# chenxuhao/GraphMiner

Measured on AMD Instinct MI355X. Metric: million edges processed/sec + total match count, higher is better.
Workload: dtype int32 (vertex ids, offsets; uint64 counts); 1 GPU; tc: triangle counting, LiveJournal stand-in; graph=rmat_s22_ef10_seed42, nv=4194304, ne_sym=81171116, tasks=40585558, max_degree=777, parallelism=task-chunk round-robin x1, replicated CSR

## Files before the change

graphminer_amd/csrc/gm_tch.hip:

```cpp
#include <type_traits>
#include "gm_flat.h"

namespace gm {

#ifndef GM_TCH_TILES
#define GM_TCH_TILES 4
#endif
constexpr int kTchTiles = GM_TCH_TILES;
#ifndef GM_TCH_TILES_SMALL
#define GM_TCH_TILES_SMALL 2
#endif
constexpr int kTchTilesSmall = GM_TCH_TILES_SMALL;
constexpr int kTchFlatTilesSmall = 4, kTchFlatTilesBig = 8;

#ifndef GM_TCH_LONG_LIST
#define GM_TCH_LONG_LIST 384
#endif
constexpr int kTchLongList = GM_TCH_LONG_LIST;

constexpr int kTchOvfCap = 128;
constexpr unsigned kTchEmpty = 0xffffffffu, kTchMarker = 0xfffffffeu;
constexpr unsigned kTchMul = 0x9E3779B1u;

template <int BITWIN>
struct alignas(16) TchWave {
  int2 desc[GM_WAVE];
  unsigned bits[BITWIN / 32 + 8];
};

#ifndef GM_TCH_WAVES_BIG
#define GM_TCH_WAVES_BIG 4
#endif
#ifndef GM_TCH_MIN_WG_BIG
#define GM_TCH_MIN_WG_BIG 4
#endif
template <int STAGE>
constexpr int tch_waves() { return STAGE <= 1024 ? kWavesPerBlock : GM_TCH_WAVES_BIG; }
template <int STAGE>
struct alignas(16) TchLds {
  uint4 table[STAGE];
  int rpl[kMaxChunkVerts + 1];
  int trpl[kMaxChunkVerts + 1];
  static constexpr int kBitWindow = STAGE <= 1024 ? 8192 : 4096;
  TchWave<kBitWindow> w[tch_waves<STAGE>()];
  int ovf_key[kTchOvfCap];
  int ovf_salt[kTchOvfCap];
  int n_ovf;
  int next_batch;
  unsigned queue_pos;
  int next_group;
};
static_assert(kTchOvfCap == 2 * GM_WAVE, "the surplus list is scanned two entries per lane");

template <int STAGE>
struct TchHash {
  static constexpr int LB = STAGE == 1024 ? 10 : 11;
  static_assert((1 << LB) == STAGE, "one bucket per stage entry");
  static constexpr unsigned kMask = (unsigned)(STAGE - 1) << 4;
  static __device__ __forceinline__ unsigned bucket(int x, unsigned s) { return ((((unsigned)x * kTchMul) >> (28 - LB)) & kMask) ^ s; }
  static __device__ __forceinline__ unsigned salt(int local_row) { return (((unsigned)local_row * 37u) & (unsigned)(STAGE - 1)) << 4; }
  static __device__ __forceinline__ int row_of(unsigned s) { return (int)(((s >> 4) * 941u) & (unsigned)(STAGE - 1)); }
};

__device__ __forceinline__ int tch_local_row(const int *rpl, const int nvl, const int e) {
  int lo = 0, hi = nvl - 1;
  while (lo < hi) {
    const int mid = (lo + hi + 1) >> 1;
    if (rpl[mid] <= e) lo = mid; else hi = mid - 1;
  }
  return lo;
}

template <int STAGE, int T>
__device__ __forceinline__ void tch_probe(const TchLds<STAGE> &B, const int *__restrict__ col, const bool fallback, const int (&key)[T],
                                          const unsigned (&salt)[T], const unsigned long long (&inm)[T], unsigned long long (&hm)[T],
                                          unsigned long long (&nm)[T]) {
  if (fallback) {
#pragma unroll
    for (int q = 0; q < T; ++q) {
      bool f = false;
      if (__builtin_amdgcn_inverse_ballot_w64(inm[q])) {
        const int lo = TchHash<STAGE>::row_of(salt[q]);
        const int rs = B.rpl[lo], rn = B.rpl[lo + 1] - rs;
        const int pos = lower_bound(col + rs, rn, key[q]);
        f = pos < rn && col[rs + pos] == key[q];
      }
      hm[q] = __ballot(f);
      nm[q] = 0ull;
    }
    return;
  }
  uint4 w[T];
#pragma unroll
  for (int q = 0; q < T; ++q)
    w[q] = *reinterpret_cast<const uint4 *>(reinterpret_cast<const char *>(B.table) + TchHash<STAGE>::bucket(key[q], salt[q]));
#pragma unroll
  for (int q = 0; q < T; ++q) {
    const unsigned k = (unsigned)key[q];
    const unsigned long long m = __ballot(w[q].x == k) | __ballot(w[q].y == k) | __ballot(w[q].z == k) | __ballot(w[q].w == k);
    hm[q] = m & inm[q];
    nm[q] = __ballot(w[q].w == kTchMarker) & ~m & inm[q];
  }
}

template <int STAGE, int T>
__device__ __forceinline__ unsigned tch_surplus(const TchLds<STAGE> &B, const int lane, const int (&key)[T], const unsigned (&salt)[T],
                                                const unsigned long long (&nm)[T]) {
  const int k0 = B.ovf_key[lane], k1 = B.ovf_key[lane + GM_WAVE];
  const int s0 = B.ovf_salt[lane], s1 = B.ovf_salt[lane + GM_WAVE];
  unsigned c = 0;
#pragma unroll
  for (int q = 0; q < T; ++q) {
    unsigned long long rest = nm[q];
    while (rest) {
      const int src = __ffsll((long long)rest) - 1;
      rest &= rest - 1;
      const int k = readlane(key[q], src), s = readlane((int)salt[q], src);
      if (__ballot(((k0 == k) & (s0 == s)) | ((k1 == k) & (s1 == s))) != 0ull) ++c;
    }
  }
  return c;
}

template <int STAGE>
__device__ __forceinline__ unsigned tch_pass(TchLds<STAGE> &B, TchWave<TchLds<STAGE>::kBitWindow> &L, const int *__restrict__ col, const bool fallback, const int lane,
                                             const int llen_all, const int key_base, const unsigned salt_l) {
  constexpr int T = STAGE <= 1024 ? kTchTilesSmall : kTchTiles;
  constexpr int TF = STAGE <= 1024 ? kTchFlatTilesSmall : kTchFlatTilesBig;
  unsigned cnt = 0;
  if (wave_max_nonneg(llen_all) == 0) return 0u;
  const bool is_long = llen_all >= kTchLongList;
  const int llen = is_long ? 0 : llen_all;

  unsigned long long lm = __ballot(is_long);
  while (lm) {
    const int src = __ffsll((long long)lm) - 1;
    lm &= lm - 1;
    const int base = readlane(key_base, src);
    const int n = readlane(llen_all, src);
    const unsigned s_u = (unsigned)readlane((int)salt_l, src);
    const int *__restrict__ kp = col + base;
    auto process = [&](auto kc, const int (&key)[T], const unsigned long long (&inm)[T]) {
      constexpr int K = decltype(kc)::value;
      int k2[K];
      unsigned salt[K];
      unsigned long long i2[K], hm[K], nm[K];
#pragma unroll
      for (int q = 0; q < K; ++q) {
        k2[q] = key[q];
        salt[q] = s_u;
        i2[q] = inm[q];
      }
      tch_probe<STAGE, K>(B, col, fallback, k2, salt, i2, hm, nm);
      unsigned long long any_need = 0ull;
#pragma unroll
      for (int q = 0; q < K; ++q) {
        cnt += (unsigned)__popcll(hm[q]);
        any_need |= nm[q];
      }
      if (any_need != 0ull) cnt += tch_surplus<STAGE, K>(B, lane, k2, salt, nm);
    };
    constexpr int G = GM_WAVE * T;
    int nxt[T];
#pragma unroll
    for (int q = 0; q < T; ++q) nxt[q] = kp[min(q * GM_WAVE + lane, n - 1)];
    int t = 0;
    for (; t + 2 * G <= n; t += G) {
      int key[T];
      unsigned long long inm[T];
#pragma unroll
      for (int q = 0; q < T; ++q) {
        key[q] = nxt[q];
        inm[q] = ~0ull;
      }
      const int *__restrict__ kn = kp + (t + G);
#pragma unroll
      for (int q = 0; q < T; ++q) nxt[q] = kn[(unsigned)(q * GM_WAVE + lane)];
      process(std::integral_constant<int, T>{}, key, inm);
    }
    for (; t < n; t += G) {
      int key[T];
      unsigned long long inm[T];
#pragma unroll
      for (int q = 0; q < T; ++q) {
        key[q] = nxt[q];
        inm[q] = __ballot((t + q * GM_WAVE + lane) < n);
      }
#pragma unroll
      for (int q = 0; q < T; ++q) nxt[q] = kp[min(t + G + q * GM_WAVE + lane, n - 1)];
      const int tiles = min(T, (n - t + GM_WAVE - 1) >> 6);
      if (tiles >= T) process(std::integral_constant<int, T>{}, key, inm);
      else if (tiles == 1) process(std::integral_constant<int, 1>{}, key, inm);
      else if constexpr (T > 2) {
        if (tiles == 2) process(std::integral_constant<int, 2>{}, key, inm);
        else process(std::integral_constant<int, (T > 2 ? 3 : 1)>{}, key, inm);
      }
    }
  }

  const int incl = wave_incl_scan_add(llen);
  const int total = readlane(incl, GM_WAVE - 1);
  if (total == 0) return cnt;
  const int off = incl - llen;
  const unsigned long long nzm = __ballot(llen > 0);
  if (llen > 0) L.desc[rank_below(nzm)] = make_int2(key_base - off, (int)salt_l);
  constexpr int G = GM_WAVE * TF, kBitWin = TchLds<STAGE>::kBitWindow;
  constexpr int TH = 4, NH = TF / TH;
  static_assert(TF % TH == 0, "tile groups are made of half-groups of four");
  struct Grp {
    int key[NH][TH];
    unsigned salt[NH][TH];
    unsigned long long inm[NH][TH];
  };
  for (int wb = 0; wb < total; wb += kBitWin) {
    const int wn = min(kBitWin, total - wb);
    const int nw = ((wn + G - 1) / G) * (G / 32) + 2;
    for (int i = lane; i < nw; i += GM_WAVE) L.bits[i] = 0u;
    wave_sync();
    if (llen > 0 && off > wb && off < wb + kBitWin) atomicOr(&L.bits[(off - 1 - wb) >> 5], 1u << ((off - 1 - wb) & 31));
    int carry = __popcll(__ballot(llen > 0 && off <= wb)) - 1;
    wave_sync();
    auto stage_a = [&](const int g, Grp &r) {
      int2 d[TF];
      bool in[TF];
      const int mw = (int)L.bits[((g * G) >> 5) + (lane & (2 * TF - 1))];
#pragma unroll
      for (int q = 0; q < TF; ++q) {
        const unsigned long long m = ((unsigned long long)(unsigned)readlane(mw, 2 * q + 1) << 32) | (unsigned)readlane(mw, 2 * q);
        const int own = carry + rank_below(m);
        carry += __popcll(m);
        in[q] = (wb + g * G + q * GM_WAVE + lane) < total;
        r.inm[q / TH][q % TH] = __ballot(in[q]);
        d[q] = L.desc[in[q] ? own : 0];
      }
#pragma unroll
      for (int q = 0; q < TF; ++q) {
        r.key[q / TH][q % TH] = col[in[q] ? d[q].x + (wb + g * G + q * GM_WAVE + lane) : 0];
        r.salt[q / TH][q % TH] = (unsigned)d[q].y;
      }
    };
    auto stage_b = [&](const Grp &r) {
#pragma unroll
      for (int h = 0; h < NH; ++h) {
        unsigned long long hm[TH], nm[TH];
        tch_probe<STAGE, TH>(B, col, fallback, r.key[h], r.salt[h], r.inm[h], hm, nm);
        unsigned long long any_need = 0ull;
#pragma unroll
        for (int q = 0; q < TH; ++q) {
          cnt += (unsigned)__popcll(hm[q]);
          any_need |= nm[q];
        }
        if (any_need != 0ull) cnt += tch_surplus<STAGE, TH>(B, lane, r.key[h], r.salt[h], nm);
      }
    };
    const int ng = (wn + G - 1) / G;
    Grp cur;
    stage_a(0, cur);
    for (int g = 0; g + 1 < ng; ++g) {
      Grp nxt;
      stage_a(g + 1, nxt);
      stage_b(cur);
      cur = nxt;
    }
    stage_b(cur);
    wave_sync();
  }
  return cnt;
}

#ifndef GM_TCH_MIN_WG
#define GM_TCH_MIN_WG 6
#endif
template <int STAGE>
__global__ __launch_bounds__((tch_waves<STAGE>() * GM_WAVE), (STAGE <= 1024 ? GM_TCH_MIN_WG : GM_TCH_MIN_WG_BIG))
void tch_kernel(const MineParams p) {
  __shared__ TchLds<STAGE> B;
  using H = TchHash<STAGE>;
  const int lane = threadIdx.x & (GM_WAVE - 1);
  const int wave = threadIdx.x >> 6;
  constexpr int nthreads = tch_waves<STAGE>() * GM_WAVE;
  const int tid = threadIdx.x;
  const int *__restrict__ rp = p.g.rp;
  const int *__restrict__ col = p.g.col;
  const int *__restrict__ trp = p.g.trp;
  const int2 *__restrict__ tdesc = p.g.tdesc;
  auto &L = B.w[wave];
  unsigned long long c0 = 0;
  for (;;) {
    if (tid == 0) B.queue_pos = atomicAdd(p.queue, (unsigned)p.grab);
    __syncthreads();
    const unsigned q = B.queue_pos;
    if (q >= (unsigned)p.count) break;
    const unsigned qe = min(q + (unsigned)p.grab, (unsigned)p.count);
    constexpr int kU = 4;
    auto chunk_at = [&](const unsigned ci) {
      const size_t pos = (size_t)p.first + (size_t)ci * (size_t)p.step;
      return p.chunks[p.order ? (size_t)p.order[pos] : pos];
    };
    ChunkRec rn = chunk_at(q);
    bool have_pre = false;
    int xn[kU], rpn = 0, trpn = 0;
    for (unsigned ci = q; ci < qe; ++ci) {
      const ChunkRec r = rn;
      const int ub = r.u_begin, nvl = r.u_end - r.u_begin;
      const int eb = r.e_begin, nel = r.e_end - r.e_begin;
      unsigned *fill32 = reinterpret_cast<unsigned *>(&B.w[0]);
      if (have_pre) {
        if (tid <= nvl) {
          B.rpl[tid] = rpn;
          B.trpl[tid] = trpn;
        }
        for (int i = tid + nthreads; i <= nvl; i += nthreads) {
          B.rpl[i] = rp[ub + i];
          B.trpl[i] = trp[ub + i];
        }
      } else {
        for (int i = tid; i <= nvl; i += nthreads) {
          B.rpl[i] = rp[ub + i];
          B.trpl[i] = trp[ub + i];
        }
      }
      {
        const uint4 empty = make_uint4(kTchEmpty, kTchEmpty, kTchEmpty, kTchEmpty);
        for (int i = tid; i < STAGE; i += nthreads) B.table[i] = empty;
        for (int i = tid; i < STAGE / 2; i += nthreads) fill32[i] = 0u;
        if (tid < kTchOvfCap) {
          B.ovf_key[tid] = -1;
          B.ovf_salt[tid] = -1;
        }
        if (tid == 0) {
          B.n_ovf = 0;
          B.next_batch = 0;
          B.next_group = 0;
        }
      }
      __syncthreads();
      unsigned *slots = reinterpret_cast<unsigned *>(B.table);
      for (int i0 = tid; i0 < nel; i0 += kU * nthreads) {
        int x[kU];
        if (have_pre && i0 == tid) {
#pragma unroll
          for (int j = 0; j < kU; ++j) x[j] = xn[j];
        } else {
#pragma unroll
          for (int j = 0; j < kU; ++j) x[j] = col[eb + min(i0 + j * nthreads, nel - 1)];
        }
#pragma unroll
        for (int j = 0; j < kU; ++j) {
          const int i = i0 + j * nthreads;
          if (i < nel) {
            const unsigned s = H::salt(tch_local_row(B.rpl, nvl, eb + i));
            const unsigned b = H::bucket(x[j], s) >> 4;
            const unsigned shift = (b & 1u) * 16u;
            const unsigned slot = (atomicAdd(&fill32[b >> 1], 1u << shift) >> shift) & 0xffffu;
            if (slot < 4u) {
              slots[(b << 2) + slot] = (unsigned)x[j];
            } else {
              const int jo = atomicAdd(&B.n_ovf, 1);
              if (jo < kTchOvfCap) {
                B.ovf_key[jo] = x[j];
                B.ovf_salt[jo] = (int)s;
              }
            }
          }
        }
      }
      __syncthreads();
      for (int b = tid; b < STAGE; b += nthreads) {
        const unsigned c = (fill32[b >> 1] >> ((b & 1) * 16)) & 0xffffu;
        if (c > 4u) {
          const unsigned x3 = slots[(b << 2) + 3];
          const int jo = atomicAdd(&B.n_ovf, 1);
          if (jo < kTchOvfCap) {
            B.ovf_key[jo] = (int)x3;
            B.ovf_salt[jo] = (int)(H::bucket((int)x3, 0u) ^ ((unsigned)b << 4));
          }
          slots[(b << 2) + 3] = kTchMarker;
        }
      }
      __syncthreads();
      const bool fallback = B.n_ovf > kTchOvfCap || (p.flags & (1 << 22)) != 0;
      have_pre = ci + 1 < qe;
      if (have_pre) {
        rn = chunk_at(ci + 1);
        const int nel_n = rn.e_end - rn.e_begin, nvl_n = rn.u_end - rn.u_begin;
#pragma unroll
        for (int j = 0; j < kU; ++j) xn[j] = col[rn.e_begin + min(tid + j * nthreads, max(nel_n - 1, 0))];
        rpn = rp[rn.u_begin + min(tid, nvl_n)];
        trpn = trp[rn.u_begin + min(tid, nvl_n)];
      }
      if (p.g.kst != nullptr) {
        constexpr int TS = 4, GS = TS * GM_WAVE;
        const int kb = p.g.kst_rp[ub], kn = p.g.kst_rp[ub + nvl] - kb;
        const unsigned *__restrict__ kp = p.g.kst + kb;
        auto grab = [&]() {
          int gi = 0;
          if (lane == 0) gi = atomicAdd(&B.next_group, 1);
          return (readfirst(gi) * r.nparts + r.part) * GS;
        };
        unsigned nxt[TS];
        int g0 = kn > 0 ? grab() : 0;
        if (g0 < kn) {
#pragma unroll
          for (int q = 0; q < TS; ++q) nxt[q] = kp[min(g0 + q * GM_WAVE + lane, kn - 1)];
        }
        while (g0 < kn) {
          const int gc = g0;
          int key[TS];
          unsigned salt[TS];
          unsigned long long inm[TS], hm[TS], nm[TS];
#pragma unroll
          for (int q = 0; q < TS; ++q) {
            key[q] = (int)(nxt[q] & 0xffffffu);
            salt[q] = H::salt((int)(((nxt[q] >> 24) - (unsigned)ub) & 255u));
            inm[q] = __ballot(gc + q * GM_WAVE + lane < kn);
          }
          g0 = grab();
          if (g0 < kn) {
#pragma unroll
            for (int q = 0; q < TS; ++q) nxt[q] = kp[min(g0 + q * GM_WAVE + lane, kn - 1)];
          }
          tch_probe<STAGE, TS>(B, col, fallback, key, salt, inm, hm, nm);
          unsigned long long any_need = 0ull;
          unsigned cnt = 0;
#pragma unroll
          for (int q = 0; q < TS; ++q) {
            cnt += (unsigned)__popcll(hm[q]);
            any_need |= nm[q];
          }
          if (any_need != 0ull) cnt += tch_surplus<STAGE, TS>(B, lane, key, salt, nm);
          c0 += (unsigned long long)cnt;
        }
      }
      const int tb = B.trpl[0], ntask = B.trpl[nvl] - tb;
      for (;;) {
        int bi = 0;
        if (lane == 0) bi = atomicAdd(&B.next_batch, 1);
        bi = readfirst(bi) * r.nparts + r.part;
        const int t0 = bi * GM_WAVE;
        if (t0 >= ntask) break;
        const bool valid = t0 + lane < ntask;
        const int te = tb + min(t0 + lane, ntask - 1);
        const int2 d = tdesc[te];
        const int lo = tch_local_row(B.trpl, nvl, te);
        const int ru = B.rpl[lo], a = B.rpl[lo + 1] - ru;
        const bool act = valid && d.y > 0 && a > 0;
        c0 += (unsigned long long)tch_pass<STAGE>(B, L, col, fallback, lane, act ? d.y : 0, d.x, H::salt(lo));
      }
      __syncthreads();
    }
  }
  if (lane == 0 && c0) atomicAdd(&p.counters[0], c0);
}

int tch_per_cu(int stage) {
  if (stage <= 1024) return 6;
  return (int)std::max<size_t>(1, std::min<size_t>(163840 / sizeof(TchLds<kTctStageMax>), 2048 / (tch_waves<kTctStageMax>() * GM_WAVE)));
}
hipError_t launch_tch(const MineParams &p, int stage, int grid_blocks, hipStream_t stream) {
  static_assert(sizeof(TchLds<1024>) * 6 <= 163840, "six workgroups per CU");
  static_assert(sizeof(TchLds<kTctStageMax>) <= 163840, "one workgroup per CU at least");
  static_assert(sizeof(TchWave<4096>) * tch_waves<kTctStageMax>() >= (size_t)kTctStageMax * 2, "fill counters alias the wave scratch");
  if (p.g.trp == nullptr || p.g.tdesc == nullptr) return hipErrorInvalidValue;
  const dim3 grid((unsigned)grid_blocks);
  if (stage <= 1024) hipLaunchKernelGGL((tch_kernel<1024>), grid, dim3(kWavesPerBlock * GM_WAVE), 0, stream, p);
  else hipLaunchKernelGGL((tch_kernel<kTctStageMax>), grid, dim3(tch_waves<kTctStageMax>() * GM_WAVE), 0, stream, p);
  return hipGetLastError();
}

}

__global__ void gm_touch_tch_kernel() {}
void gm_touch_tch() { hipLaunchKernelGGL(gm_touch_tch_kernel, dim3(1), dim3(1), 0, 0); }
```

Before: 23930 Medges/s.

## Precompute hash buckets, narrow 32-bit col offsets, and drop per-lane bounds checks in TC probes

Callers now pass precomputed LDS bucket offsets to the probe, and the salt is redefined as the global host id, so tagged keys map straight to a bucket without per-key salt arithmetic. A NARROW template variant, used when the edge count fits in 29 bits, keeps column offsets as biased 32-bit byte offsets instead of 64-bit addresses. Descriptor lookup uses mbcnt directly, and only the final partial tile group is guarded. The flat loop is unrolled into two ping-pong buffers, and the key-group prefetch skips clamping for full groups. This lowers VALU and address work per probe, at the cost of more kernel instantiations and trickier offset and bias arithmetic.

Result: slower. 20080 Medges/s (-16.1%).

```diff
diff --git a/graphminer_amd/csrc/gm_tch.hip b/graphminer_amd/csrc/gm_tch.hip
--- a/graphminer_amd/csrc/gm_tch.hip
+++ b/graphminer_amd/csrc/gm_tch.hip
@@ -58,8 +58,12 @@
   static_assert((1 << LB) == STAGE, "one bucket per stage entry");
   static constexpr unsigned kMask = (unsigned)(STAGE - 1) << 4;
   static __device__ __forceinline__ unsigned bucket(int x, unsigned s) { return ((((unsigned)x * kTchMul) >> (28 - LB)) & kMask) ^ s; }
-  static __device__ __forceinline__ unsigned salt(int local_row) { return (((unsigned)local_row * 37u) & (unsigned)(STAGE - 1)) << 4; }
-  static __device__ __forceinline__ int row_of(unsigned s) { return (int)(((s >> 4) * 941u) & (unsigned)(STAGE - 1)); }
+  static constexpr int kSaltShift = LB - 4;
+  static __device__ __forceinline__ unsigned salt(int host) { return ((unsigned)host & 255u) << kSaltShift; }
+  static __device__ __forceinline__ int row_of(unsigned s, int ub) { return (int)(((s >> kSaltShift) - (unsigned)ub) & 255u); }
+  static __device__ __forceinline__ unsigned bucket_tagged(unsigned w) {
+    return ((((w & 0xffffffu) * kTchMul) ^ (w & 0xff000000u)) >> (28 - LB)) & kMask;
+  }
 };
 
 __device__ __forceinline__ int tch_local_row(const int *rpl, const int nvl, const int e) {
@@ -72,15 +76,15 @@
 }
 
 template <int STAGE, int T>
-__device__ __forceinline__ void tch_probe(const TchLds<STAGE> &B, const int *__restrict__ col, const bool fallback, const int (&key)[T],
-                                          const unsigned (&salt)[T], const unsigned long long (&inm)[T], unsigned long long (&hm)[T],
+__device__ __forceinline__ void tch_probe(const TchLds<STAGE> &B, const int *__restrict__ col, const bool fallback, const int ub, const int (&key)[T],
+                                          const unsigned (&bkt)[T], const unsigned long long (&inm)[T], unsigned long long (&hm)[T],
                                           unsigned long long (&nm)[T]) {
   if (fallback) {
 #pragma unroll
     for (int q = 0; q < T; ++q) {
       bool f = false;
       if (__builtin_amdgcn_inverse_ballot_w64(inm[q])) {
-        const int lo = TchHash<STAGE>::row_of(salt[q]);
+        const int lo = TchHash<STAGE>::row_of(bkt[q] ^ TchHash<STAGE>::bucket(key[q], 0u), ub);
         const int rs = B.rpl[lo], rn = B.rpl[lo + 1] - rs;
         const int pos = lower_bound(col + rs, rn, key[q]);
         f = pos < rn && col[rs + pos] == key[q];
@@ -92,8 +96,7 @@
   }
   uint4 w[T];
 #pragma unroll
-  for (int q = 0; q < T; ++q)
-    w[q] = *reinterpret_cast<const uint4 *>(reinterpret_cast<const char *>(B.table) + TchHash<STAGE>::bucket(key[q], salt[q]));
+  for (int q = 0; q < T; ++q) w[q] = *reinterpret_cast<const uint4 *>(reinterpret_cast<const char *>(B.table) + bkt[q]);
 #pragma unroll
   for (int q = 0; q < T; ++q) {
     const unsigned k = (unsigned)key[q];
@@ -104,7 +107,7 @@
 }
 
 template <int STAGE, int T>
-__device__ __forceinline__ unsigned tch_surplus(const TchLds<STAGE> &B, const int lane, const int (&key)[T], const unsigned (&salt)[T],
+__device__ __forceinline__ unsigned tch_surplus(const TchLds<STAGE> &B, const int lane, const int (&key)[T], const unsigned (&bkt)[T],
                                                 const unsigned long long (&nm)[T]) {
   const int k0 = B.ovf_key[lane], k1 = B.ovf_key[lane + GM_WAVE];
   const int s0 = B.ovf_salt[lane], s1 = B.ovf_salt[lane + GM_WAVE];
@@ -115,16 +118,17 @@
     while (rest) {
       const int src = __ffsll((long long)rest) - 1;
       rest &= rest - 1;
-      const int k = readlane(key[q], src), s = readlane((int)salt[q], src);
+      const int k = readlane(key[q], src);
+      const int s = (int)((unsigned)readlane((int)bkt[q], src) ^ TchHash<STAGE>::bucket(k, 0u));
       if (__ballot(((k0 == k) & (s0 == s)) | ((k1 == k) & (s1 == s))) != 0ull) ++c;
     }
   }
   return c;
 }
 
-template <int STAGE>
-__device__ __forceinline__ unsigned tch_pass(TchLds<STAGE> &B, TchWave<TchLds<STAGE>::kBitWindow> &L, const int *__restrict__ col, const bool fallback, const int lane,
-                                             const int llen_all, const int key_base, const unsigned salt_l) {
+template <int STAGE, bool NARROW>
+__device__ __forceinline__ unsigned tch_pass(TchLds<STAGE> &B, TchWave<TchLds<STAGE>::kBitWindow> &L, const int *__restrict__ col, const bool fallback, const int ub,
+                                             const int lane, const int llen_all, const int key_base, const unsigned salt_l) {
   constexpr int T = STAGE <= 1024 ? kTchTilesSmall : kTchTiles;
   constexpr int TF = STAGE <= 1024 ? kTchFlatTilesSmall : kTchFlatTilesBig;
   unsigned cnt = 0;
@@ -143,22 +147,22 @@
     auto process = [&](auto kc, const int (&key)[T], const unsigned long long (&inm)[T]) {
       constexpr int K = decltype(kc)::value;
       int k2[K];
-      unsigned salt[K];
+      unsigned bk[K];
       unsigned long long i2[K], hm[K], nm[K];
 #pragma unroll
       for (int q = 0; q < K; ++q) {
         k2[q] = key[q];
-        salt[q] = s_u;
+        bk[q] = TchHash<STAGE>::bucket(key[q], s_u);
         i2[q] = inm[q];
       }
-      tch_probe<STAGE, K>(B, col, fallback, k2, salt, i2, hm, nm);
+      tch_probe<STAGE, K>(B, col, fallback, ub, k2, bk, i2, hm, nm);
       unsigned long long any_need = 0ull;
 #pragma unroll
       for (int q = 0; q < K; ++q) {
         cnt += (unsigned)__popcll(hm[q]);
         any_need |= nm[q];
       }
-      if (any_need != 0ull) cnt += tch_surplus<STAGE, K>(B, lane, k2, salt, nm);
+      if (any_need != 0ull) cnt += tch_surplus<STAGE, K>(B, lane, k2, bk, nm);
     };
     constexpr int G = GM_WAVE * T;
     int nxt[T];
@@ -203,8 +207,10 @@
   if (total == 0) return cnt;
   const int off = incl - llen;
   const unsigned long long nzm = __ballot(llen > 0);
-  if (llen > 0) L.desc[rank_below(nzm)] = make_int2(key_base - off, (int)salt_l);
   constexpr int G = GM_WAVE * TF, kBitWin = TchLds<STAGE>::kBitWindow;
+  constexpr unsigned kBias = (unsigned)(GM_WAVE * (TF - 1)) << 2;
+  if (llen > 0) L.desc[rank_below(nzm)] = make_int2(NARROW ? (int)(((unsigned)(key_base - off) << 2) + kBias) : key_base - off, (int)salt_l);
+  const char *__restrict__ cbase = reinterpret_cast<const char *>(col) - kBias;
   constexpr int TH = 4, NH = TF / TH;
   static_assert(TF % TH == 0, "tile groups are made of half-groups of four");
   struct Grp {
@@ -212,6 +218,7 @@
     unsigned salt[NH][TH];
     unsigned long long inm[NH][TH];
   };
+  const unsigned lane4 = (unsigned)lane << 2;
   for (int wb = 0; wb < total; wb += kBitWin) {
     const int wn = min(kBitWin, total - wb);
     const int nw = ((wn + G - 1) / G) * (G / 32) + 2;
@@ -222,47 +229,74 @@
     wave_sync();
     auto stage_a = [&](const int g, Grp &r) {
       int2 d[TF];
-      bool in[TF];
+      const int p0 = wb + g * G;
       const int mw = (int)L.bits[((g * G) >> 5) + (lane & (2 * TF - 1))];
 #pragma unroll
       for (int q = 0; q < TF; ++q) {
-        const unsigned long long m = ((unsigned long long)(unsigned)readlane(mw, 2 * q + 1) << 32) | (unsigned)readlane(mw, 2 * q);
-        const int own = carry + rank_below(m);
-        carry += __popcll(m);
-        in[q] = (wb + g * G + q * GM_WAVE + lane) < total;
-        r.inm[q / TH][q % TH] = __ballot(in[q]);
-        d[q] = L.desc[in[q] ? own : 0];
-      }
+        const unsigned mlo = (unsigned)readlane(mw, 2 * q), mhi = (unsigned)readlane(mw, 2 * q + 1);
+        const int2 *dp = L.desc + carry;
+        d[q] = dp[__builtin_amdgcn_mbcnt_hi(mhi, __builtin_amdgcn_mbcnt_lo(mlo, 0u))];
+        carry += __popc(mlo) + __popc(mhi);
+        r.salt[q / TH][q % TH] = (unsigned)d[q].y;
+        r.inm[q / TH][q % TH] = ~0ull;
+      }
+      using Off = std::conditional_t<NARROW, unsigned, long long>;
+      Off o[TF];
 #pragma unroll
       for (int q = 0; q < TF; ++q) {
-        r.key[q / TH][q % TH] = col[in[q] ? d[q].x + (wb + g * G + q * GM_WAVE + lane) : 0];
-        r.salt[q / TH][q % TH] = (unsigned)d[q].y;
+        if constexpr (NARROW) o[q] = (unsigned)d[q].x + (lane4 + (unsigned)(p0 << 2));
+        else o[q] = (long long)d[q].x + (long long)(p0 + q * GM_WAVE + lane);
+      }
+      if (p0 + G > total) {
+        asm volatile("; guarded tile group");
+#pragma unroll
+        for (int q = 0; q < TF; ++q) {
+          const int n = max(min(total - (p0 + q * GM_WAVE), GM_WAVE), 0);
+          const unsigned long long m = n >= GM_WAVE ? ~0ull : ((1ull << n) - 1ull);
+          r.inm[q / TH][q % TH] = m;
+          o[q] = __builtin_amdgcn_inverse_ballot_w64(m) ? o[q] : (Off)(NARROW ? kBias - (unsigned)(q * GM_WAVE * 4) : 0u);
+        }
+      }
+#pragma unroll
+      for (int q = 0; q < TF; ++q) {
+        if constexpr (NARROW) r.key[q / TH][q % TH] = *reinterpret_cast<const int *>(cbase + (size_t)o[q] + (size_t)(q * GM_WAVE * 4));
+        else r.key[q / TH][q % TH] = col[o[q]];
       }
     };
     auto stage_b = [&](const Grp &r) {
 #pragma unroll
       for (int h = 0; h < NH; ++h) {
+        unsigned bk[TH];
         unsigned long long hm[TH], nm[TH];
-        tch_probe<STAGE, TH>(B, col, fallback, r.key[h], r.salt[h], r.inm[h], hm, nm);
+#pragma unroll
+        for (int q = 0; q < TH; ++q) bk[q] = TchHash<STAGE>::bucket(r.key[h][q], r.salt[h][q]);
+        tch_probe<STAGE, TH>(B, col, fallback, ub, r.key[h], bk, r.inm[h], hm, nm);
         unsigned long long any_need = 0ull;
 #pragma unroll
         for (int q = 0; q < TH; ++q) {
           cnt += (unsigned)__popcll(hm[q]);
           any_need |= nm[q];
         }
-        if (any_need != 0ull) cnt += tch_surplus<STAGE, TH>(B, lane, r.key[h], r.salt[h], nm);
+        if (any_need != 0ull) cnt += tch_surplus<STAGE, TH>(B, lane, r.key[h], bk, nm);
       }
     };
     const int ng = (wn + G - 1) / G;
-    Grp cur;
-    stage_a(0, cur);
-    for (int g = 0; g + 1 < ng; ++g) {
-      Grp nxt;
-      stage_a(g + 1, nxt);
-      stage_b(cur);
-      cur = nxt;
+    Grp ga, gb;
+    stage_a(0, ga);
+    for (int g = 0;; g += 2) {
+      if (g + 1 >= ng) {
+        stage_b(ga);
+        break;
+      }
+      stage_a(g + 1, gb);
+      stage_b(ga);
+      if (g + 2 >= ng) {
+        stage_b(gb);
+        break;
+      }
+      stage_a(g + 2, ga);
+      stage_b(gb);
     }
-    stage_b(cur);
     wave_sync();
   }
   return cnt;
@@ -271,13 +305,13 @@
 #ifndef GM_TCH_MIN_WG
 #define GM_TCH_MIN_WG 6
 #endif
-template <int STAGE>
+template <int STAGE, bool NARROW>
 __global__ __launch_bounds__((tch_waves<STAGE>() * GM_WAVE), (STAGE <= 1024 ? GM_TCH_MIN_WG : GM_TCH_MIN_WG_BIG))
 void tch_kernel(const MineParams p) {
   __shared__ TchLds<STAGE> B;
   using H = TchHash<STAGE>;
   const int lane = threadIdx.x & (GM_WAVE - 1);
-  const int wave = threadIdx.x >> 6;
+  const int wave = readfirst((int)(threadIdx.x >> 6));
   constexpr int nthreads = tch_waves<STAGE>() * GM_WAVE;
   const int tid = threadIdx.x;
   const int *__restrict__ rp = p.g.rp;
@@ -349,7 +383,7 @@
         for (int j = 0; j < kU; ++j) {
           const int i = i0 + j * nthreads;
           if (i < nel) {
-            const unsigned s = H::salt(tch_local_row(B.rpl, nvl, eb + i));
+            const unsigned s = H::salt(ub + tch_local_row(B.rpl, nvl, eb + i));
             const unsigned b = H::bucket(x[j], s) >> 4;
             const unsigned shift = (b & 1u) * 16u;
             const unsigned slot = (atomicAdd(&fill32[b >> 1], 1u << shift) >> shift) & 0xffffu;
@@ -399,28 +433,44 @@
           return (readfirst(gi) * r.nparts + r.part) * GS;
         };
         unsigned nxt[TS];
-        int g0 = kn > 0 ? grab() : 0;
-        if (g0 < kn) {
-#pragma unroll
-          for (int q = 0; q < TS; ++q) nxt[q] = kp[min(g0 + q * GM_WAVE + lane, kn - 1)];
+        auto request = [&](const int g) {
+          if (g + GS <= kn) {
+            const unsigned *__restrict__ kg = kp + g;
+#pragma unroll
+            for (int q = 0; q < TS; ++q) nxt[q] = kg[(unsigned)(q * GM_WAVE + lane)];
+          } else {
+#pragma unroll
+            for (int q = 0; q < TS; ++q) nxt[q] = kp[min(g + q * GM_WAVE + lane, kn - 1)];
+            asm volatile("; guarded tile group");
+          }
+        };
+        int g0 = kn;
+        if (kn > 0) {
+          g0 = grab();
+          request(g0);
         }
         while (g0 < kn) {
           const int gc = g0;
           int key[TS];
-          unsigned salt[TS];
+          unsigned bk[TS];
           unsigned long long inm[TS], hm[TS], nm[TS];
 #pragma unroll
           for (int q = 0; q < TS; ++q) {
             key[q] = (int)(nxt[q] & 0xffffffu);
-            salt[q] = H::salt((int)(((nxt[q] >> 24) - (unsigned)ub) & 255u));
-            inm[q] = __ballot(gc + q * GM_WAVE + lane < kn);
+            bk[q] = H::bucket_tagged(nxt[q]);
+            inm[q] = ~0ull;
+          }
+          if (gc + GS > kn) {
+            asm volatile("; guarded tile group");
+#pragma unroll
+            for (int q = 0; q < TS; ++q) {
+              const int n = max(min(kn - (gc + q * GM_WAVE), GM_WAVE), 0);
+              inm[q] = n >= GM_WAVE ? ~0ull : ((1ull << n) - 1ull);
+            }
           }
           g0 = grab();
-          if (g0 < kn) {
-#pragma unroll
-            for (int q = 0; q < TS; ++q) nxt[q] = kp[min(g0 + q * GM_WAVE + lane, kn - 1)];
-          }
-          tch_probe<STAGE, TS>(B, col, fallback, key, salt, inm, hm, nm);
+          request(g0);
+          tch_probe<STAGE, TS>(B, col, fallback, ub, key, bk, inm, hm, nm);
           unsigned long long any_need = 0ull;
           unsigned cnt = 0;
 #pragma unroll
@@ -428,7 +478,7 @@
             cnt += (unsigned)__popcll(hm[q]);
             any_need |= nm[q];
           }
-          if (any_need != 0ull) cnt += tch_surplus<STAGE, TS>(B, lane, key, salt, nm);
+          if (any_need != 0ull) cnt += tch_surplus<STAGE, TS>(B, lane, key, bk, nm);
           c0 += (unsigned long long)cnt;
         }
       }
@@ -445,7 +495,7 @@
         const int lo = tch_local_row(B.trpl, nvl, te);
         const int ru = B.rpl[lo], a = B.rpl[lo + 1] - ru;
         const bool act = valid && d.y > 0 && a > 0;
-        c0 += (unsigned long long)tch_pass<STAGE>(B, L, col, fallback, lane, act ? d.y : 0, d.x, H::salt(lo));
+        c0 += (unsigned long long)tch_pass<STAGE, NARROW>(B, L, col, fallback, ub, lane, act ? d.y : 0, d.x, H::salt(ub + lo));
       }
       __syncthreads();
     }
@@ -463,8 +513,12 @@
   static_assert(sizeof(TchWave<4096>) * tch_waves<kTctStageMax>() >= (size_t)kTctStageMax * 2, "fill counters alias the wave scratch");
   if (p.g.trp == nullptr || p.g.tdesc == nullptr) return hipErrorInvalidValue;
   const dim3 grid((unsigned)grid_blocks);
-  if (stage <= 1024) hipLaunchKernelGGL((tch_kernel<1024>), grid, dim3(kWavesPerBlock * GM_WAVE), 0, stream, p);
-  else hipLaunchKernelGGL((tch_kernel<kTctStageMax>), grid, dim3(tch_waves<kTctStageMax>() * GM_WAVE), 0, stream, p);
+  const bool narrow = (unsigned)p.g.ne < (1u << 29);
+  const dim3 small(kWavesPerBlock * GM_WAVE), big(tch_waves<kTctStageMax>() * GM_WAVE);
+  if (stage <= 1024 && narrow) hipLaunchKernelGGL((tch_kernel<1024, true>), grid, small, 0, stream, p);
+  else if (stage <= 1024) hipLaunchKernelGGL((tch_kernel<1024, false>), grid, small, 0, stream, p);
+  else if (narrow) hipLaunchKernelGGL((tch_kernel<kTctStageMax, true>), grid, big, 0, stream, p);
+  else hipLaunchKernelGGL((tch_kernel<kTctStageMax, false>), grid, big, 0, stream, p);
   return hipGetLastError();
 }
 
```
